# genomematt/xenomapper

Hardware: AMD Instinct MI355X
Metric: read-pairs/sec classified (higher is better)
Workload: dtype int32; 1 GPU; configs[1]: 50000000 PE 2x150 pairs/GPU, AS/XS, liberal, HBM-resident; pairs_per_gpu=50000000, step=xm_classify_compact_dev: classify+count, scan, scatter (3 launches)

## Files before the change

### xenomapper_amd/csrc/xm_api.hip

```cpp
#include <hip/hip_runtime.h>
#include <stdint.h>
#include <stdio.h>
#include <stdlib.h>
#include <string.h>

#include <dlfcn.h>

#include <string>
#include <vector>

#include <rccl/rccl.h>

#include "xm_kernels.h"
#include "xm_pinned.h"

struct TimedSpan {
    int kernel;
    hipEvent_t start, stop;
};

struct xm_ctx {
    int device;
    int n_cu;
    char name[128];
    uint32_t max_blocks;
    uint32_t *d_gran_counts;
    uint32_t *d_gran_off;
    uint64_t *d_counts_rep;
    uint32_t *d_part_tot;
    hipStream_t ws_stream;
    bool ws_used, ws_released;
    hipEvent_t ws_event;
    void *d_scratch[8];
    size_t scratch_bytes[8];
    bool timing;
    uint32_t timing_mask;
    std::vector<TimedSpan> spans;
    std::vector<hipEvent_t> free_events;
    double acc_ms[XM_K_COUNT];
    uint64_t acc_launches[XM_K_COUNT];
    std::string last_error;
    ncclComm_t comm;
    int comm_ranks;
// ... 112 lines not shown
int order_workspace(xm_ctx *ctx, hipStream_t st)
{
    if (capturing(st)) return XM_OK;
    if (ctx->ws_released) {
        XM_HIP(ctx, hipStreamWaitEvent(st, ctx->ws_event, 0));
        ctx->ws_released = false;
    } else if (ctx->ws_used && ctx->ws_stream != st && !capturing(ctx->ws_stream)) {
        XM_HIP(ctx, hipEventRecord(ctx->ws_event, ctx->ws_stream));
        XM_HIP(ctx, hipStreamWaitEvent(st, ctx->ws_event, 0));
    }
    ctx->ws_stream = st;
    ctx->ws_used = true;
    return XM_OK;
}

}

extern "C" {

int xm_abi_version(void) { return XM_ABI_VERSION; }

const char *xm_strerror(int status)
{
    switch (status) {
    case XM_OK: return "ok";
    case XM_ERR_INVALID_ARG: return "invalid argument";
    case XM_ERR_NO_DEVICE: return "no usable gfx950 (MI355X) device";
    case XM_ERR_HIP: return "HIP runtime error";
    case XM_ERR_OOM: return "out of device memory";
    case XM_ERR_RANGE: return "CIGAR-derived score outside int32";
// ... 17 lines not shown
    if (strncmp(prop.gcnArchName, "gfx950", 6) != 0) {
        char buf[200];
        snprintf(buf, sizeof buf, "device %d is %s, not gfx950", device_id, prop.gcnArchName);
        return no_device(buf, hipSuccess);
    }
    if ((he = hipSetDevice(device_id)) != hipSuccess) return no_device("hipSetDevice", he);

    xm_ctx *ctx = new xm_ctx();
    ctx->device = device_id;
    ctx->n_cu = prop.multiProcessorCount;
    snprintf(ctx->name, sizeof ctx->name, "%s (%s)", prop.name, prop.gcnArchName);
    ctx->max_blocks = (uint32_t)ctx->n_cu * 8u;
    ctx->d_gran_counts = nullptr;
    ctx->d_gran_off = nullptr;
    ctx->d_counts_rep = nullptr;
    ctx->d_part_tot = nullptr;
    ctx->ws_stream = nullptr;
    ctx->ws_used = false;
    ctx->ws_released = false;
    ctx->ws_event = nullptr;
    for (int i = 0; i < 8; ++i) { ctx->d_scratch[i] = nullptr; ctx->scratch_bytes[i] = 0; }
    ctx->timing = false;
    ctx->comm = nullptr;
    ctx->comm_ranks = 0;
    ctx->timing_mask = ~0u;
    for (int k = 0; k < XM_K_COUNT; ++k) { ctx->acc_ms[k] = 0.0; ctx->acc_launches[k] = 0; }
    const size_t ws = ((size_t)XM_MAX_GRANULES + 64) * 8 * sizeof(uint32_t);
    hipError_t e = hipMalloc((void **)&ctx->d_gran_counts, ws);
    if (e == hipSuccess) e = hipMalloc((void **)&ctx->d_gran_off, ws);
    if (e == hipSuccess) e = hipMalloc((void **)&ctx->d_counts_rep, COUNTS_REP_BYTES);
// ... 16 lines not shown
}

int xm_ctx_destroy(xm_ctx *ctx)
{
    if (!ctx) return XM_ERR_INVALID_ARG;
    (void)hipSetDevice(ctx->device);
    (void)hipDeviceSynchronize();
    if (ctx->comm) (void)xm_comm_destroy(ctx);
    for (auto &sp : ctx->spans) { (void)hipEventDestroy(sp.start); (void)hipEventDestroy(sp.stop); }
    for (auto &e : ctx->free_events) (void)hipEventDestroy(e);
    for (int i = 0; i < 8; ++i)
        if (ctx->d_scratch[i]) (void)hipFree(ctx->d_scratch[i]);
    (void)hipFree(ctx->d_gran_counts);
    (void)hipFree(ctx->d_gran_off);
    (void)hipFree(ctx->d_counts_rep);
    (void)hipFree(ctx->d_part_tot);
    (void)hipEventDestroy(ctx->ws_event);
    delete ctx;
    return XM_OK;
}

int xm_ctx_device_info(const xm_ctx *ctx, int *n_cu, char *name, size_t name_len)
{
    if (!ctx) return XM_ERR_INVALID_ARG;
    if (n_cu) *n_cu = ctx->n_cu;
    if (name && name_len) snprintf(name, name_len, "%s", ctx->name);
    return XM_OK;
}


// ... 109 lines not shown
        xm::launch_scan(st, cp, ctx->d_gran_off, bin_totals, counts);
    }
    if ((rc = check_launch(ctx, "scan_kernel")) != XM_OK) {
        reset_count_state(ctx, st);
        return rc;
    }
    {
        Span span(ctx, st, XM_K_SCATTER);
        xm::launch_scatter(st, cp.plan, mode, n, from_bins4 ? cp.bins4 : code, from_bins4, cp.gran_counts, ctx->d_gran_off,
                           bin_totals, bin_offsets, idx_out, ctx->d_part_tot, lists, cp.gran0, cp.gran1);
    }
    if ((rc = check_launch(ctx, "scatter_kernel")) != XM_OK) reset_count_state(ctx, st);
    return rc;
}

static xm::CountPlan count_plan(xm_ctx *ctx, uint64_t n)
{
    xm::CountPlan cp;
    cp.plan = xm::plan_granules(n);
    cp.gran_counts = ctx->d_gran_counts;
    cp.counts_rep = ctx->d_counts_rep;
    cp.part_tot = ctx->d_part_tot;
    cp.bins4 = nullptr;
    return cp;
}

static int empty_compact(xm_ctx *ctx, hipStream_t st, uint64_t *bin_offsets, uint64_t *counts)
{
    XM_HIP(ctx, hipMemsetAsync(counts, 0, 64 * sizeof(uint64_t), st));
    XM_HIP(ctx, hipMemsetAsync(bin_offsets, 0, 8 * sizeof(uint64_t), st));
    return XM_OK;
}

int xm_compact_dev(xm_ctx *ctx, void *stream, int mode, uint64_t n, const uint8_t *code,
                   uint32_t *idx_out, uint64_t *bin_offsets, uint64_t *counts)
{
    if (!ctx || bad_mode(mode) || n > XM_MAX_RECORDS || wrong_device(ctx)) return XM_ERR_INVALID_ARG;
    if (!bin_offsets || !counts) return XM_ERR_INVALID_ARG;
    hipStream_t st = (hipStream_t)stream;
    if (n == 0) return empty_compact(ctx, st, bin_offsets, counts);
    if (!code || !idx_out || ((uintptr_t)code & 15u)) return XM_ERR_INVALID_ARG;
    const xm::CountPlan cp = count_plan(ctx, n);
    int rc;
    if ((rc = order_workspace(ctx, st)) != XM_OK) return rc;
    {
        Span span(ctx, st, XM_K_HIST);
        xm::launch_hist(st, mode, n, code, cp);
    }
    if ((rc = check_launch(ctx, "hist_kernel")) != XM_OK) return rc;
    return compact_tail(ctx, st, mode, n, code, cp, idx_out, bin_offsets, counts);
}


int xm_classify_compact_dev(xm_ctx *ctx, void *stream, int mode, uint64_t n,
                            const int32_t *as1, const int32_t *xs1, const int32_t *as2, const int32_t *xs2,
                            const uint64_t *unit_bits, int32_t min_score_floor, uint8_t *code_out, uint8_t *bins4,
                            uint32_t *idx_out, uint64_t *bin_offsets, uint64_t *counts)
{
    if (!ctx || bad_mode(mode) || n > XM_MAX_RECORDS || wrong_device(ctx)) return XM_ERR_INVALID_ARG;
    if (!bin_offsets || !counts) return XM_ERR_INVALID_ARG;
    hipStream_t st = (hipStream_t)stream;
    if (n == 0) return empty_compact(ctx, st, bin_offsets, counts);
    if (!as1 || !xs1 || !as2 || !xs2 || !unit_bits || (!code_out && !bins4) || !idx_out) return XM_ERR_INVALID_ARG;
    if ((((uintptr_t)as1 | (uintptr_t)xs1 | (uintptr_t)as2 | (uintptr_t)xs2 | (uintptr_t)code_out | (uintptr_t)bins4) & 15u))
        return XM_ERR_INVALID_ARG;
    xm::CountPlan cp = count_plan(ctx, n);
    cp.bins4 = bins4;
    int rc;
    if ((rc = order_workspace(ctx, st)) != XM_OK) return rc;
    {
        Span span(ctx, st, XM_K_CLASSIFY);
        xm::launch_classify_i32(st, mode, n, as1, xs1, as2, xs2, unit_bits, min_score_floor, code_out, &cp);
    }
    if ((rc = check_launch(ctx, "classify_kernel<int32, counts>")) != XM_OK) return rc;
    return compact_tail(ctx, st, mode, n, code_out, cp, idx_out, bin_offsets, counts);
}

int xm_classify_compact_f64_dev(xm_ctx *ctx, void *stream, int mode, uint64_t n,
                                const double *as1, const double *xs1, const double *as2, const double *xs2,
                                const uint64_t *unit_bits, double min_score, uint8_t *code_out, uint8_t *bins4,
                                uint32_t *idx_out, uint64_t *bin_offsets, uint64_t *counts)
{
    if (!ctx || bad_mode(mode) || n > XM_MAX_RECORDS || wrong_device(ctx)) return XM_ERR_INVALID_ARG;
    if (!bin_offsets || !counts) return XM_ERR_INVALID_ARG;
    hipStream_t st = (hipStream_t)stream;
    if (n == 0) return empty_compact(ctx, st, bin_offsets, counts);
    if (!as1 || !xs1 || !as2 || !xs2 || !unit_bits || (!code_out && !bins4) || !idx_out) return XM_ERR_INVALID_ARG;
    if ((((uintptr_t)as1 | (uintptr_t)xs1 | (uintptr_t)as2 | (uintptr_t)xs2) & 31u) || (((uintptr_t)code_out | (uintptr_t)bins4) & 15u))
        return XM_ERR_INVALID_ARG;
    xm::CountPlan cp = count_plan(ctx, n);
    cp.bins4 = bins4;
    int rc;
    if ((rc = order_workspace(ctx, st)) != XM_OK) return rc;
    {
        Span span(ctx, st, XM_K_CLASSIFY);
        xm::launch_classify_f64(st, mode, n, as1, xs1, as2, xs2, unit_bits, min_score, code_out, &cp);
    }
    if ((rc = check_launch(ctx, "classify_kernel<f64, counts>")) != XM_OK) return rc;
    return compact_tail(ctx, st, mode, n, code_out, cp, idx_out, bin_offsets, counts);
}

int xm_classify_compact_cigar_dev(xm_ctx *ctx, void *stream, int mode, uint64_t n,
                                  const int32_t *nm1, const uint32_t *off1, const uint32_t *ops1, const int32_t *xs1,
                                  const int32_t *nm2, const uint32_t *off2, const uint32_t *ops2, const int32_t *xs2,
                                  const uint64_t *unit_bits, int32_t min_score_floor, uint8_t *code_out,
                                  uint32_t *range_flag, uint32_t *idx_out, uint64_t *bin_offsets, uint64_t *counts)
{
    if (!ctx || bad_mode(mode) || n > XM_MAX_RECORDS || wrong_device(ctx)) return XM_ERR_INVALID_ARG;
// ... 21 lines not shown
                                         const int32_t *nm2, const uint8_t *cnt2, const uint32_t *tile2, const uint32_t *ops2,
                                         const int32_t *xs2,
                                         const uint64_t *unit_bits, int32_t min_score_floor, uint8_t *code_out, uint8_t *bins4,
                                         uint32_t *range_flag, uint32_t *idx_out, uint64_t *bin_offsets, uint64_t *counts)
{
    if (!ctx || bad_mode(mode) || n > XM_MAX_RECORDS || wrong_device(ctx)) return XM_ERR_INVALID_ARG;
    if (!bin_offsets || !counts) return XM_ERR_INVALID_ARG;
    hipStream_t st = (hipStream_t)stream;
    if (n == 0) return empty_compact(ctx, st, bin_offsets, counts);
    if (!nm1 || !cnt1 || !tile1 || !ops1 || !xs1 || !nm2 || !cnt2 || !tile2 || !ops2 || !xs2 || !unit_bits ||
        (!code_out && !bins4) || !idx_out)
        return XM_ERR_INVALID_ARG;
    if ((((uintptr_t)nm1 | (uintptr_t)xs1 | (uintptr_t)nm2 | (uintptr_t)xs2 | (uintptr_t)code_out | (uintptr_t)bins4) & 15u) ||
        (((uintptr_t)cnt1 | (uintptr_t)cnt2 | (uintptr_t)tile1 | (uintptr_t)tile2 | (uintptr_t)ops1 | (uintptr_t)ops2) & 3u))
        return XM_ERR_INVALID_ARG;
    xm::CountPlan cp = count_plan(ctx, n);
    cp.bins4 = bins4;
    const xm::CigCols s1 = {nm1, xs1, cnt1, tile1, ops1}, s2 = {nm2, xs2, cnt2, tile2, ops2};
    int rc;
    if ((rc = order_workspace(ctx, st)) != XM_OK) return rc;
    {
        Span span(ctx, st, XM_K_CLASSIFY);
        xm::launch_classify_cigp(st, mode, n, s1, s2, unit_bits, min_score_floor, code_out, range_flag, cp);
    }
    if ((rc = check_launch(ctx, "classify_cigp_kernel")) != XM_OK) return rc;
    return compact_tail(ctx, st, mode, n, code_out, cp, idx_out, bin_offsets, counts);
}


static int list_out(uint32_t *const idx_out[6], uint32_t *idx_state6, uint64_t list_capacity, xm::ListOut &lo)
{
    if (!idx_out) return XM_ERR_INVALID_ARG;
    for (int b = 0; b < 6; ++b) {
        if (!idx_out[b] || ((uintptr_t)idx_out[b] & 3u)) return XM_ERR_INVALID_ARG;
        lo.p[b] = idx_out[b];
// ... 41 lines not shown
int xm_classify_place_dev(xm_ctx *ctx, void *stream, int mode, uint64_t n,
                          const int32_t *as1, const int32_t *xs1, const int32_t *as2, const int32_t *xs2,
                          const uint64_t *unit_bits, int32_t min_score_floor, uint8_t *code_out, uint8_t *bins4,
                          uint32_t *const idx_out[6], uint64_t list_capacity, uint64_t *n_out, uint64_t *counts)
{
    if (!ctx || bad_mode(mode) || n > XM_MAX_RECORDS || wrong_device(ctx)) return XM_ERR_INVALID_ARG;
    if (!n_out || !counts) return XM_ERR_INVALID_ARG;
    xm::ListOut lo;
    int rc;
    if ((rc = list_out(idx_out, nullptr, list_capacity, lo)) != XM_OK) return rc;
    hipStream_t st = (hipStream_t)stream;
    if (n == 0) return empty_compact(ctx, st, n_out, counts);
    if (!as1 || !xs1 || !as2 || !xs2 || !unit_bits || (!code_out && !bins4)) return XM_ERR_INVALID_ARG;
    if ((((uintptr_t)as1 | (uintptr_t)xs1 | (uintptr_t)as2 | (uintptr_t)xs2 | (uintptr_t)code_out | (uintptr_t)bins4) & 15u))
        return XM_ERR_INVALID_ARG;
    xm::CountPlan cp = count_plan(ctx, n);
    cp.bins4 = bins4;
    if ((rc = order_workspace(ctx, st)) != XM_OK) return rc;
    return place_steps(ctx, st, mode, n, cp, code_out, lo, n_out, counts, "classify_kernel<int32, counts>", [&](const xm::CountPlan &c) {
        xm::launch_classify_i32(st, mode, n, as1, xs1, as2, xs2, unit_bits, min_score_floor, code_out, &c);
    });
}

int xm_classify_place_f64_dev(xm_ctx *ctx, void *stream, int mode, uint64_t n,
                              const double *as1, const double *xs1, const double *as2, const double *xs2,
                              const uint64_t *unit_bits, double min_score, uint8_t *code_out, uint8_t *bins4,
                              uint32_t *const idx_out[6], uint32_t *idx_state6, uint64_t list_capacity,
                              uint64_t *n_out, uint64_t *counts)
{
    if (!ctx || bad_mode(mode) || n > XM_MAX_RECORDS || wrong_device(ctx)) return XM_ERR_INVALID_ARG;
    if (!n_out || !counts) return XM_ERR_INVALID_ARG;
    xm::ListOut lo;
    int rc;
    if ((rc = list_out(idx_out, idx_state6, list_capacity, lo)) != XM_OK) return rc;
    hipStream_t st = (hipStream_t)stream;
    if (n == 0) return empty_compact(ctx, st, n_out, counts);
    if (!as1 || !xs1 || !as2 || !xs2 || !unit_bits || (!code_out && !bins4)) return XM_ERR_INVALID_ARG;
    if ((((uintptr_t)as1 | (uintptr_t)xs1 | (uintptr_t)as2 | (uintptr_t)xs2) & 31u) || (((uintptr_t)code_out | (uintptr_t)bins4) & 15u))
        return XM_ERR_INVALID_ARG;
    xm::CountPlan cp = count_plan(ctx, n);
    cp.bins4 = bins4;
    if ((rc = order_workspace(ctx, st)) != XM_OK) return rc;
    return place_steps(ctx, st, mode, n, cp, code_out, lo, n_out, counts, "classify_kernel<f64, counts>", [&](const xm::CountPlan &c) {
        xm::launch_classify_f64(st, mode, n, as1, xs1, as2, xs2, unit_bits, min_score, code_out, &c);
    });
}

int xm_classify_place_cigar_packed_dev(xm_ctx *ctx, void *stream, int mode, uint64_t n,
                                       const int32_t *nm1, const uint8_t *cnt1, const uint32_t *tile1, const uint32_t *ops1,
                                       const int32_t *xs1,
                                       const int32_t *nm2, const uint8_t *cnt2, const uint32_t *tile2, const uint32_t *ops2,
                                       const int32_t *xs2,
                                       const uint64_t *unit_bits, int32_t min_score_floor, uint8_t *code_out, uint8_t *bins4,
                                       uint32_t *range_flag, uint32_t *const idx_out[6], uint64_t list_capacity,
                                       uint64_t *n_out, uint64_t *counts)
{
    if (!ctx || bad_mode(mode) || n > XM_MAX_RECORDS || wrong_device(ctx)) return XM_ERR_INVALID_ARG;
    if (!n_out || !counts) return XM_ERR_INVALID_ARG;
    xm::ListOut lo;
    int rc;
    if ((rc = list_out(idx_out, nullptr, list_capacity, lo)) != XM_OK) return rc;
    hipStream_t st = (hipStream_t)stream;
    if (n == 0) return empty_compact(ctx, st, n_out, counts);
    if (!nm1 || !cnt1 || !tile1 || !ops1 || !xs1 || !nm2 || !cnt2 || !tile2 || !ops2 || !xs2 || !unit_bits || (!code_out && !bins4))
        return XM_ERR_INVALID_ARG;
    if ((((uintptr_t)nm1 | (uintptr_t)xs1 | (uintptr_t)nm2 | (uintptr_t)xs2 | (uintptr_t)code_out | (uintptr_t)bins4) & 15u) ||
        (((uintptr_t)cnt1 | (uintptr_t)cnt2 | (uintptr_t)tile1 | (uintptr_t)tile2 | (uintptr_t)ops1 | (uintptr_t)ops2) & 3u))
        return XM_ERR_INVALID_ARG;
    xm::CountPlan cp = count_plan(ctx, n);
    cp.bins4 = bins4;
    const xm::CigCols s1 = {nm1, xs1, cnt1, tile1, ops1}, s2 = {nm2, xs2, cnt2, tile2, ops2};
    if ((rc = order_workspace(ctx, st)) != XM_OK) return rc;
    {
        Span span(ctx, st, XM_K_CLASSIFY);
        xm::launch_classify_cigp(st, mode, n, s1, s2, unit_bits, min_score_floor, code_out, range_flag, cp);
    }
    if ((rc = check_launch(ctx, "classify_cigp_kernel")) != XM_OK) return rc;
    return compact_tail(ctx, st, mode, n, code_out, cp, nullptr, n_out, counts, &lo);
}


static int runs_common(xm_ctx *ctx, hipStream_t st, int mode, uint64_t n, size_t elem,
                       const void *as1, const void *xs1, const void *as2, const void *xs2, const uint64_t *unit_bits,
                       int32_t mi, double mf, uint16_t *runs16, uint16_t *gran_counts, uint64_t *n_out, uint64_t *counts)
{
    if (!ctx || bad_mode(mode) || n > XM_MAX_RECORDS || wrong_device(ctx)) return XM_ERR_INVALID_ARG;
    if (!n_out || !counts) return XM_ERR_INVALID_ARG;
// ... 139 lines not shown
    XM_HIP(ctx, hipSetDevice(ctx->device));
    const size_t col_bytes = (size_t)n * elem;
    const size_t bits_bytes = (size_t)((n + 63) / 64) * 8;
    const void *src[4] = {as1, xs1, as2, xs2};
    int rc;
    for (int c = 0; c < 4; ++c) {
        if ((rc = ensure_scratch(ctx, c, col_bytes)) != XM_OK) return rc;
        XM_HIP(ctx, hipMemcpy(ctx->d_scratch[c], src[c], col_bytes, hipMemcpyHostToDevice));
    }
    if ((rc = ensure_scratch(ctx, 4, bits_bytes)) != XM_OK) return rc;
    XM_HIP(ctx, hipMemcpy(ctx->d_scratch[4], unit_bits, bits_bytes, hipMemcpyHostToDevice));
    if ((rc = ensure_scratch(ctx, 5, (size_t)n + 16)) != XM_OK) return rc;
    if ((rc = ensure_scratch(ctx, 7, 72 * sizeof(uint64_t))) != XM_OK) return rc;
    uint8_t *d_code = (uint8_t *)ctx->d_scratch[5];
    uint64_t *d_counts = (uint64_t *)ctx->d_scratch[7] + 8;
    const xm::CountPlan cp = count_plan(ctx, n);
    if (counts && (rc = order_workspace(ctx, nullptr)) != XM_OK) return rc;
    {
        Span span(ctx, nullptr, XM_K_CLASSIFY);
        if (elem == 4)
            xm::launch_classify_i32(nullptr, mode, n, (const int32_t *)ctx->d_scratch[0], (const int32_t *)ctx->d_scratch[1],
                                    (const int32_t *)ctx->d_scratch[2], (const int32_t *)ctx->d_scratch[3],
                                    (const uint64_t *)ctx->d_scratch[4], mi, d_code, counts ? &cp : nullptr);
        else
            xm::launch_classify_f64(nullptr, mode, n, (const double *)ctx->d_scratch[0], (const double *)ctx->d_scratch[1],
                                    (const double *)ctx->d_scratch[2], (const double *)ctx->d_scratch[3],
                                    (const uint64_t *)ctx->d_scratch[4], mf, d_code, counts ? &cp : nullptr);
    }
    if ((rc = check_launch(ctx, "classify_kernel")) != XM_OK) return rc;
    if (counts) {
        if ((rc = counts_only_tail(ctx, cp, d_counts)) != XM_OK) return rc;
        XM_HIP(ctx, hipMemcpy(counts, d_counts, 64 * sizeof(uint64_t), hipMemcpyDeviceToHost));
// ... 531 lines not shown
```

### xenomapper_amd/csrc/xm_kernels.h

```cpp
#pragma once
#include <hip/hip_runtime.h>
#include <stdint.h>

#include "../../include/xenomapper_hip.h"

#define XM_BLOCK 256
#define XM_GRAN 2048
#define XM_MAX_GRANULES ((uint32_t)((0xFFFFF000ull + XM_GRAN - 1) / XM_GRAN))
#define XM_PART_GRAN 1024u
#define XM_PART_STRIDE 2112u
#define XM_PART_REPLICAS 64u
#define XM_COUNT_REPLICAS 64u
#define XM_CLASSIFY_BLOCK 512
#ifndef XM_CIGAR_BLOCK
#define XM_CIGAR_BLOCK 256
#endif
#define XM_CIGP_BLOCK 512
#ifndef XM_SCATTER_WAVES
#define XM_SCATTER_WAVES 1048576u
#endif
#define XM_CLASSIFY_NT true

namespace xm {

struct GranPlan {
    uint32_t n_gran;
    uint32_t gran_stride;
};

struct CountPlan {
    GranPlan plan = {0, 0};
    uint32_t *gran_counts = nullptr;
    uint32_t *part_tot = nullptr;
    uint8_t *bins4 = nullptr;
    uint64_t *counts_rep = nullptr;
    uint32_t gran0 = 0, gran1 = 0;
};

GranPlan plan_granules(uint64_t n);

struct CigCols {
    const int32_t *nm;
    const int32_t *xs;
    const uint8_t *cnt;
    const uint32_t *tile;
    const uint32_t *ops;
};

struct ListOut {
    uint32_t *p[7];
// ... 41 lines not shown
```

### xenomapper_amd/csrc/xm_kernels.hip

```cpp
#include <hip/hip_runtime.h>
#include <stdint.h>
#include <stdlib.h>

#include "xm_kernels.h"

namespace xm {

template <typename T>
__device__ __forceinline__ uint32_t mapping_state(T a1, T x1, T a2, T x2, T m)
{
    const bool low1 = a1 <= m;
    const bool low2 = a2 <= m;
    const bool prim = (a1 > m) && (low2 || a1 > a2);
    const bool sec  = (a2 > m) && (low1 || a2 > a1);
    const bool spec1 = (x1 == T(0)) || (a1 > x1);
    const bool spec2 = (x2 == T(0)) || (a2 > x2);
    uint32_t s = 6u;
    s = sec ? (spec2 ? 1u : 3u) : s;
    s = (a1 == a2) ? 4u : s;
    s = prim ? (spec1 ? 0u : 2u) : s;
    s = (low1 && low2) ? 5u : s;
    return s;
}

// ... 79 lines not shown
{
    return (uint32_t)__builtin_amdgcn_readlane((int)v, lane);
}

__device__ __forceinline__ void lds_settle()
{
    asm volatile("s_waitcnt lgkmcnt(0)" ::: "memory");
}

#define XM_HREP 8
#define XM_COUNT_LDS_WORDS (64 * XM_HREP + 16)

struct CountSink {
    uint32_t *gran_counts;
    uint32_t *part_tot;
    unsigned long long *counts_rep;
    uint8_t *bins4;
    uint32_t gran_stride;
    int mode;
    uint32_t blk0;
};

__device__ __forceinline__ void count_flush(uint32_t *lds, uint32_t granule, const CountSink &sink)
{
    const uint32_t lane = threadIdx.x & 63u;
    uint32_t *misc = lds + 64 * XM_HREP;
    const uint4 h0 = *reinterpret_cast<const uint4 *>(lds + lane * XM_HREP);
    const uint4 h1 = *reinterpret_cast<const uint4 *>(lds + lane * XM_HREP + 4);
    const uint32_t s = h0.x + h0.y + h0.z + h0.w + h1.x + h1.y + h1.z + h1.w;
    if (s != 0u) {
        atomicAdd(&sink.counts_rep[(granule % XM_COUNT_REPLICAS) * 64u + lane], (unsigned long long)s);
        atomicAdd(&misc[8u + bin_of_code(sink.mode, lane)], s);
    }
    lds_settle();
    if (lane < 8u) {
        const uint32_t v = misc[8u + lane];
        sink.gran_counts[(uint64_t)lane * sink.gran_stride + granule] = v;
        if (v != 0u) atomicAdd(&sink.part_tot[((granule & (XM_PART_REPLICAS - 1u)) * 8u + lane) * XM_PART_STRIDE + granule / XM_PART_GRAN], v);
    }
}

template <int BLOCK>
__device__ __forceinline__ void count_units(const uint32_t c[4], uint32_t *lds, const CountSink &sink)
{
    const uint32_t lane = threadIdx.x & 63u;
    const uint32_t rep = lane & (XM_HREP - 1u);
#pragma unroll
    for (int j = 0; j < 4; ++j) {
// ... 221 lines not shown
{
    v += __shfl_xor(v, 1, 64);  v += __shfl_xor(v, 2, 64);  v += __shfl_xor(v, 4, 64);
    v += __shfl_xor(v, 8, 64);  v += __shfl_xor(v, 16, 64); v += __shfl_xor(v, 32, 64);
    if ((threadIdx.x & 63u) == 0u) wsum[threadIdx.x >> 6] = v;
    __syncthreads();
    unsigned long long total = 0;
#pragma unroll
    for (int w = 0; w < XM_SCAN_THREADS / 64; ++w) total += wsum[w];
    return total;
}

__global__ void __launch_bounds__(XM_SCAN_THREADS)
scan_kernel(const uint32_t *__restrict__ gran_counts, uint32_t n_gran, uint32_t gran_stride,
            const uint32_t *__restrict__ part_tot, uint32_t *__restrict__ gran_off,
            unsigned long long *__restrict__ bin_totals,
            unsigned long long *__restrict__ counts_rep, unsigned long long *__restrict__ counts, uint32_t part0, uint32_t n_parts)
{
    __shared__ unsigned long long wsum[XM_SCAN_THREADS / 64];
    __shared__ uint32_t wtot[XM_SCAN_THREADS / 64];
    const uint32_t p = blockIdx.x + part0, b = blockIdx.y;
    const uint32_t t = threadIdx.x, lane = t & 63u, wave = t >> 6;
    if (p + 1u == n_parts && t < 64u) {
        const uint32_t slot = b * 8u + (t >> 3), part = t & 7u;
        unsigned long long acc = 0;
        for (uint32_t r = part; r < XM_COUNT_REPLICAS; r += 8u) {
            acc += counts_rep[r * 64u + slot];
            counts_rep[r * 64u + slot] = 0;
        }
        acc += __shfl_xor(acc, 1, 64);
        acc += __shfl_xor(acc, 2, 64);
        acc += __shfl_xor(acc, 4, 64);
        if (part == 0) counts[slot] = acc;
    }
    const uint32_t g = p * XM_PART_GRAN + t;
    const uint32_t x = (g < n_gran) ? gran_counts[(uint64_t)b * gran_stride + g] : 0u;
    unsigned long long part_sum = 0;
    for (uint32_t e = t; e < p * XM_PART_REPLICAS; e += XM_SCAN_THREADS) {
        const uint32_t r = e / p, q = e - r * p;
        part_sum += part_tot[(r * 8u + b) * XM_PART_STRIDE + q];
    }
    const unsigned long long carry = block_sum_1024(part_sum, wsum);

    const uint32_t incl = wave_scan_incl(x);
    if (lane == 63u) wtot[wave] = incl;
    __syncthreads();
    uint32_t before_wave = 0, part_total = 0;
    for (uint32_t w = 0; w < XM_SCAN_THREADS / 64; ++w) {
        const uint32_t v = wtot[w];
        before_wave += (w < wave) ? v : 0u;
        part_total += v;
    }
    if (g < n_gran) gran_off[(uint64_t)b * gran_stride + g] = (uint32_t)carry + before_wave + incl - x;
    if (p + 1u == n_parts && t == 0u) bin_totals[b] = carry + part_total;
}

#ifndef XM_SCATTER_GUARD
// ... 169 lines not shown
    __shared__ __attribute__((aligned(16))) uint16_t slab_all[CAN_STAGE ? XM_BLOCK / 64 : 1][CAN_STAGE ? XM_SLAB_U16 : 4];
    const uint32_t lane = threadIdx.x & 63u;
    if (last) {
        const uint32_t n_parts = (n_gran + XM_PART_GRAN - 1u) / XM_PART_GRAN, cells = 8u * XM_PART_REPLICAS * n_parts;
        for (uint32_t i = blockIdx.x * XM_BLOCK + threadIdx.x; i < cells; i += gridDim.x * XM_BLOCK)
            part_tot[(i / n_parts) * XM_PART_STRIDE + i % n_parts] = 0u;
    }
    const uint32_t wave = (uint32_t)__builtin_amdgcn_readfirstlane((int)(threadIdx.x >> 6));
    const uint32_t g0 = g_first + (blockIdx.x * (XM_BLOCK / 64) + wave) * (MULTI ? gran_per_wave : 1u);
    if (g0 >= n_gran) return;
    uint8_t *lut = lut_all[NIB ? 0 : wave];
    if (!NIB) lut[lane] = (uint8_t)bin_of_code(mode, lane == 63u ? XM_NO_UNIT : lane);
    uint64_t *lptr = lptr_all[LISTS ? wave : 0];
    if (LISTS && lane < 8u) lptr[lane] = lane < 7u ? (uint64_t)(uintptr_t)lo.p[lane] : 0ull;

    uint32_t lane_base, n_units;
    {
        const uint32_t tot = (lane < 8u) ? (uint32_t)bin_totals[lane] : 0u;
        const uint32_t off = (lane < 7u) ? gran_off[(uint64_t)lane * gran_stride + g0] : 0u;
        const uint32_t bin_start = wave_scan_incl(tot) - tot;
        lane_base = LISTS ? off : bin_start + off;
        n_units = LISTS ? lo.cap : lane_value(bin_start, 7);
        if (g0 == g_first && last && lane < 8u) bin_offsets[lane] = (LISTS && lane < 7u) ? tot : bin_start;
    }
    uint16_t *slab = slab_all[CAN_STAGE ? wave : 0];

    auto load_granule = [&](uint32_t g, uint32_t w[NSUB]) {
        const uint64_t rec_g = (uint64_t)g * (NSUB * 256u);
        if (NIB) {
            const uint16_t *nib = reinterpret_cast<const uint16_t *>(code) + (rec_g >> 2) + lane;
#pragma unroll
            for (int s = 0; s < NSUB; ++s) w[s] = nib[s * 64];
        } else if (rec_g + NSUB * 256u <= n) {
#pragma unroll
            for (int s = 0; s < NSUB; ++s) w[s] = *reinterpret_cast<const uint32_t *>(code + rec_g + s * 256u + lane * 4u);
        } else {
#pragma unroll
            for (int s = 0; s < NSUB; ++s) w[s] = load_codes4_tail(code, rec_g + s * 256u + lane * 4u, n);
        }
    };
    auto slab_layout = [&](uint32_t cnt_g, uint32_t &run_start, uint32_t &run_len) -> bool {
        const uint32_t room = (lane < 7u) ? ((cnt_g + 3u) & ~3u) + 4u : 0u;
        const uint32_t incl_room = wave_scan_incl(room), incl_cnt = wave_scan_incl(cnt_g);
        run_start = incl_room - room + (lane_base & 3u);
        const uint32_t cnt = lane_base < n_units ? (cnt_g < n_units - lane_base ? cnt_g : n_units - lane_base) : 0u;
        run_len = run_start < (uint32_t)XM_SLAB_U16 ? (cnt < XM_SLAB_U16 - run_start ? cnt : XM_SLAB_U16 - run_start) : 0u;
        return lane_value(incl_cnt, 6) >= (uint32_t)XM_STAGE_MIN_UNITS;
    };
    auto copy_runs_out = [&](uint32_t run_start, uint32_t run_len, uint32_t rec_g) {
#pragma unroll
        for (int b = 0; b < 7; ++b) {
            const uint32_t N = lane_value(run_len, b);
            uint32_t *__restrict__ dst = LISTS ? lo.p[b] : idx_out;
            if (N == 0u || dst == nullptr) continue;
            scatter_copy_out<WIDE>(slab, lane_value(run_start, b), lane_value(lane_base, b), N, rec_g, dst);
        }
    };

    if (!MULTI) {
        const uint32_t g = g0;
        uint32_t run_start = 0, run_len = 0;
        bool staged = false;
        if (CAN_STAGE) {
            const uint32_t cnt_g = (lane < 7u) ? gran_counts[(uint64_t)lane * gran_stride + g] : 0u;
            staged = slab_layout(cnt_g, run_start, run_len);
        }
        uint32_t base[7];
#pragma unroll
        for (int b = 0; b < 7; ++b) base[b] = lane_value(staged ? run_start : lane_base, b);
        const uint32_t rec_g = (uint32_t)((uint64_t)g * (NSUB * 256u));
        uint32_t w[NSUB];
        load_granule(g, w);
        if (!NIB || LISTS) lds_settle();
        if (CAN_STAGE && staged) {
            scatter_granule<NSUB, WIDE, NIB, true, LISTS>(w, lut, rec_g, base, idx_out, n_units, slab, lptr);
            lds_settle();
            copy_runs_out(run_start, run_len, rec_g);
        } else {
            scatter_granule<NSUB, WIDE, NIB, false, LISTS>(w, lut, rec_g, base, idx_out, n_units, slab, lptr);
        }
        return;
    }

    const uint32_t g1 = g0 + gran_per_wave < n_gran ? g0 + gran_per_wave : n_gran;
    uint32_t base[7];
#pragma unroll
    for (int b = 0; b < 7; ++b) base[b] = lane_value(lane_base, b);
    uint32_t w[NSUB], wn[NSUB];
    load_granule(g0, w);
    if (!NIB || LISTS) lds_settle();
    for (uint32_t g = g0; g < g1; ++g) {
        if (g + 1u < g1) load_granule(g + 1u, wn);
        const uint32_t rec_g = (uint32_t)((uint64_t)g * (NSUB * 256u));
        bool staged = false;
        uint32_t cnt_g = 0;
        if (CAN_STAGE) {
            cnt_g = (lane < 7u) ? gran_counts[(uint64_t)lane * gran_stride + g] : 0u;
            uint32_t run_start, run_len;
            staged = slab_layout(cnt_g, run_start, run_len);
            if (staged) {
                uint32_t sbase[7];
#pragma unroll
                for (int b = 0; b < 7; ++b) sbase[b] = lane_value(run_start, b);
                scatter_granule<NSUB, WIDE, NIB, true, LISTS>(w, lut, rec_g, sbase, idx_out, n_units, slab, lptr);
                lds_settle();
                copy_runs_out(run_start, run_len, rec_g);
                lds_settle();
            }
        }
        if (!staged) {
            if (CAN_STAGE) {
#pragma unroll
// ... 433 lines not shown
#pragma unroll
        for (int j = 0; j < 4; ++j) a1[j] = a2[j] = INT32_MIN;
    }
    if (__ballot(bad) != 0ull && (threadIdx.x & 63u) == 0u && range_flag) atomicOr(range_flag, 1u);

    uint32_t halo = 0;
    if (PAIRED && threadIdx.x == 0) {
        if (r0 > 0) {
            const uint64_t h = r0 - 1;
            halo = mapping_state<int32_t>(cigar_score_one(nm1, off1, ops1, h, range_flag), xs1[h],
                                          cigar_score_one(nm2, off2, ops2, h, range_flag), xs2[h], m);
        } else {
            mb &= ~1u;
        }
    }
    const CountSink none = {nullptr, nullptr, nullptr, nullptr, 0u, 0, 0u};
    classify_finish<int32_t, PAIRED, BLOCK, FULL, false, -1>(a1, x1, a2, x2, m, mb, halo, last_state, code, r0, n, nullptr, none);
}

template <bool PAIRED, int BLOCK>
__global__ void __launch_bounds__(BLOCK)
classify_cigar_kernel(const int32_t *__restrict__ nm1, const uint32_t *__restrict__ off1, const uint32_t *__restrict__ ops1,
                      const int32_t *__restrict__ xs1,
                      const int32_t *__restrict__ nm2, const uint32_t *__restrict__ off2, const uint32_t *__restrict__ ops2,
                      const int32_t *__restrict__ xs2,
                      const uint8_t *__restrict__ unit_bits8, int32_t m, uint8_t *__restrict__ code, uint64_t n,
                      uint32_t *__restrict__ range_flag)
{
    __shared__ uint32_t last_state[BLOCK / 64];
    __shared__ __attribute__((aligned(16))) uint32_t cig_table[BLOCK / 64][XM_CIG_WAVE_OPS + 4];
    uint32_t *cig_T = cig_table[threadIdx.x >> 6];
// ... 334 lines not shown
GranPlan plan_granules(uint64_t n)
{
    GranPlan p;
    uint64_t g = (n + XM_GRAN - 1) / XM_GRAN;
    if (g == 0) g = 1;
    p.n_gran = (uint32_t)g;
    p.gran_stride = (p.n_gran + 63u) & ~63u;
    return p;
}

static CountSink make_sink(const CountPlan *cp, int mode)
{
    CountSink s;
    s.gran_counts = cp ? cp->gran_counts : nullptr;
    s.part_tot = cp ? cp->part_tot : nullptr;
    s.counts_rep = cp ? reinterpret_cast<unsigned long long *>(cp->counts_rep) : nullptr;
    s.bins4 = cp ? cp->bins4 : nullptr;
    s.gran_stride = cp ? cp->plan.gran_stride : 0u;
    s.mode = mode;
    s.blk0 = cp ? cp->gran0 : 0u;
    return s;
}

template <typename T>
static void launch_classify_t(hipStream_t st, int mode, uint64_t n,
                              const T *as1, const T *xs1, const T *as2, const T *xs2,
                              const uint64_t *unit_bits, T m, uint8_t *code, const CountPlan *cp)
{
    const uint64_t per_block = (uint64_t)XM_CLASSIFY_BLOCK * 4;
    static_assert(XM_CLASSIFY_BLOCK * 4 == XM_GRAN, "a counting workgroup is a granule: CountPlan's chunk is in both");
    const uint32_t all = (uint32_t)((n + per_block - 1) / per_block);
// ... 99 lines not shown
        if (mode == XM_MODE_SE) XM_LAUNCH_CIGP(false, -1); else XM_LAUNCH_CIGP(true, -1);
    }
#undef XM_LAUNCH_CIGP
}

void launch_hist(hipStream_t st, int mode, uint64_t n, const uint8_t *code, const CountPlan &cp)
{
    const uint32_t grid = (cp.plan.n_gran + (XM_BLOCK / 64) - 1) / (XM_BLOCK / 64);
    hist_kernel<<<grid, XM_BLOCK, 0, st>>>(code, n, cp.plan.n_gran, make_sink(&cp, mode));
}

void launch_scan(hipStream_t st, const CountPlan &cp, uint32_t *gran_off, uint64_t *bin_totals, uint64_t *counts)
{
    const uint32_t n_parts = (cp.plan.n_gran + XM_PART_GRAN - 1) / XM_PART_GRAN;
    unsigned long long *bt = reinterpret_cast<unsigned long long *>(bin_totals);
    unsigned long long *rep = reinterpret_cast<unsigned long long *>(cp.counts_rep);
    unsigned long long *cnt = reinterpret_cast<unsigned long long *>(counts);
    const uint32_t part0 = cp.gran1 ? cp.gran0 / XM_PART_GRAN : 0u;
    const uint32_t part1 = cp.gran1 ? (cp.gran1 + XM_PART_GRAN - 1) / XM_PART_GRAN : n_parts;
    scan_kernel<<<dim3(part1 - part0, 8), XM_SCAN_THREADS, 0, st>>>(cp.gran_counts, cp.gran1 ? cp.gran1 : cp.plan.n_gran, cp.plan.gran_stride,
                                                                   cp.part_tot, gran_off, bt, rep, cnt, part0, n_parts);
}

static uint32_t scatter_waves()
{
    const char *e = getenv("XM_SCATTER_WAVES");
    const long v = e && *e ? strtol(e, nullptr, 10) : 0;
    return v >= 1 && v < (long)XM_SCATTER_WAVES ? (uint32_t)v : (uint32_t)XM_SCATTER_WAVES;
}

void launch_scatter(hipStream_t st, const GranPlan &p, int mode, uint64_t n, const uint8_t *code, bool code_is_bins4,
                    const uint32_t *gran_counts, const uint32_t *gran_off, const uint64_t *bin_totals, uint64_t *bin_offsets,
                    uint32_t *idx_out, uint32_t *part_tot, const ListOut *lists, uint32_t gran0, uint32_t gran1)
{
    const unsigned long long *bt = reinterpret_cast<const unsigned long long *>(bin_totals);
    unsigned long long *bo = reinterpret_cast<unsigned long long *>(bin_offsets);
// ... 39 lines not shown
```

Baseline: 141.8 billion read-pairs/s.

## Replace replicated 64-bit count atomics with per-granule category rows reduced in scan

The classify/count epilogue no longer does a global 64-bit atomicAdd into replicated count slots. Each granule now writes its 64 category counts as uint16 into a new per-granule workspace, and the scan kernel reduces those rows per partition with wave shuffles before one atomic per bin. The scatter kernel also hoists the first granule's code and count loads ahead of the bin-total setup so their latency overlaps. This trades global atomic contention for extra HBM traffic, a lazily grown workspace, and zeroing of counts by granule 0, which relies on classify finishing before scan.

```diff
diff --git a/xenomapper_amd/csrc/xm_api.hip b/xenomapper_amd/csrc/xm_api.hip
--- a/xenomapper_amd/csrc/xm_api.hip
+++ b/xenomapper_amd/csrc/xm_api.hip
@@ -27,6 +27,8 @@
     uint32_t *d_gran_counts;
     uint32_t *d_gran_off;
     uint64_t *d_counts_rep;
+    uint16_t *d_gran_cat;
+    uint32_t gran_cat_cap;
     uint32_t *d_part_tot;
     hipStream_t ws_stream;
     bool ws_used, ws_released;
@@ -169,6 +171,25 @@
     return XM_OK;
 }
 
+int claim_workspace(xm_ctx *ctx, hipStream_t st, xm::CountPlan &cp)
+{
+    if (cp.plan.n_gran > ctx->gran_cat_cap) {
+        if (capturing(st)) {
+            ctx->last_error = "the workspace must grow for this input: run the call once outside the capture first";
+            return XM_ERR_INVALID_ARG;
+        }
+        if (ctx->d_gran_cat) XM_HIP(ctx, hipFree(ctx->d_gran_cat));
+        ctx->d_gran_cat = nullptr;
+        ctx->gran_cat_cap = 0;
+        const uint64_t room = (uint64_t)cp.plan.n_gran + cp.plan.n_gran / 8u + 64u;
+        const uint32_t cap = room > XM_MAX_GRANULES ? XM_MAX_GRANULES : (uint32_t)room;
+        XM_HIP(ctx, hipMalloc((void **)&ctx->d_gran_cat, (size_t)cap * 64 * sizeof(uint16_t)));
+        ctx->gran_cat_cap = cap;
+    }
+    cp.gran_cat = ctx->d_gran_cat;
+    return order_workspace(ctx, st);
+}
+
 }
 
 extern "C" {
@@ -216,6 +237,8 @@
     ctx->d_gran_counts = nullptr;
     ctx->d_gran_off = nullptr;
     ctx->d_counts_rep = nullptr;
+    ctx->d_gran_cat = nullptr;
+    ctx->gran_cat_cap = 0;
     ctx->d_part_tot = nullptr;
     ctx->ws_stream = nullptr;
     ctx->ws_used = false;
@@ -262,6 +285,7 @@
     (void)hipFree(ctx->d_gran_counts);
     (void)hipFree(ctx->d_gran_off);
     (void)hipFree(ctx->d_counts_rep);
+    if (ctx->d_gran_cat) (void)hipFree(ctx->d_gran_cat);
     (void)hipFree(ctx->d_part_tot);
     (void)hipEventDestroy(ctx->ws_event);
     delete ctx;
@@ -401,12 +425,12 @@
     return rc;
 }
 
-static xm::CountPlan count_plan(xm_ctx *ctx, uint64_t n)
+static xm::CountPlan count_plan(xm_ctx *ctx, uint64_t n, uint64_t *counts)
 {
     xm::CountPlan cp;
     cp.plan = xm::plan_granules(n);
     cp.gran_counts = ctx->d_gran_counts;
-    cp.counts_rep = ctx->d_counts_rep;
+    cp.counts = counts;
     cp.part_tot = ctx->d_part_tot;
     cp.bins4 = nullptr;
     return cp;
@@ -427,9 +451,9 @@
     hipStream_t st = (hipStream_t)stream;
     if (n == 0) return empty_compact(ctx, st, bin_offsets, counts);
     if (!code || !idx_out || ((uintptr_t)code & 15u)) return XM_ERR_INVALID_ARG;
-    const xm::CountPlan cp = count_plan(ctx, n);
-    int rc;
-    if ((rc = order_workspace(ctx, st)) != XM_OK) return rc;
+    xm::CountPlan cp = count_plan(ctx, n, counts);
+    int rc;
+    if ((rc = claim_workspace(ctx, st, cp)) != XM_OK) return rc;
     {
         Span span(ctx, st, XM_K_HIST);
         xm::launch_hist(st, mode, n, code, cp);
@@ -451,10 +475,10 @@
     if (!as1 || !xs1 || !as2 || !xs2 || !unit_bits || (!code_out && !bins4) || !idx_out) return XM_ERR_INVALID_ARG;
     if ((((uintptr_t)as1 | (uintptr_t)xs1 | (uintptr_t)as2 | (uintptr_t)xs2 | (uintptr_t)code_out | (uintptr_t)bins4) & 15u))
         return XM_ERR_INVALID_ARG;
-    xm::CountPlan cp = count_plan(ctx, n);
+    xm::CountPlan cp = count_plan(ctx, n, counts);
     cp.bins4 = bins4;
     int rc;
-    if ((rc = order_workspace(ctx, st)) != XM_OK) return rc;
+    if ((rc = claim_workspace(ctx, st, cp)) != XM_OK) return rc;
     {
         Span span(ctx, st, XM_K_CLASSIFY);
         xm::launch_classify_i32(st, mode, n, as1, xs1, as2, xs2, unit_bits, min_score_floor, code_out, &cp);
@@ -475,10 +499,10 @@
     if (!as1 || !xs1 || !as2 || !xs2 || !unit_bits || (!code_out && !bins4) || !idx_out) return XM_ERR_INVALID_ARG;
     if ((((uintptr_t)as1 | (uintptr_t)xs1 | (uintptr_t)as2 | (uintptr_t)xs2) & 31u) || (((uintptr_t)code_out | (uintptr_t)bins4) & 15u))
         return XM_ERR_INVALID_ARG;
-    xm::CountPlan cp = count_plan(ctx, n);
+    xm::CountPlan cp = count_plan(ctx, n, counts);
     cp.bins4 = bins4;
     int rc;
-    if ((rc = order_workspace(ctx, st)) != XM_OK) return rc;
+    if ((rc = claim_workspace(ctx, st, cp)) != XM_OK) return rc;
     {
         Span span(ctx, st, XM_K_CLASSIFY);
         xm::launch_classify_f64(st, mode, n, as1, xs1, as2, xs2, unit_bits, min_score, code_out, &cp);
@@ -530,11 +554,11 @@
     if ((((uintptr_t)nm1 | (uintptr_t)xs1 | (uintptr_t)nm2 | (uintptr_t)xs2 | (uintptr_t)code_out | (uintptr_t)bins4) & 15u) ||
         (((uintptr_t)cnt1 | (uintptr_t)cnt2 | (uintptr_t)tile1 | (uintptr_t)tile2 | (uintptr_t)ops1 | (uintptr_t)ops2) & 3u))
         return XM_ERR_INVALID_ARG;
-    xm::CountPlan cp = count_plan(ctx, n);
+    xm::CountPlan cp = count_plan(ctx, n, counts);
     cp.bins4 = bins4;
     const xm::CigCols s1 = {nm1, xs1, cnt1, tile1, ops1}, s2 = {nm2, xs2, cnt2, tile2, ops2};
     int rc;
-    if ((rc = order_workspace(ctx, st)) != XM_OK) return rc;
+    if ((rc = claim_workspace(ctx, st, cp)) != XM_OK) return rc;
     {
         Span span(ctx, st, XM_K_CLASSIFY);
         xm::launch_classify_cigp(st, mode, n, s1, s2, unit_bits, min_score_floor, code_out, range_flag, cp);
@@ -606,9 +630,9 @@
     if (!as1 || !xs1 || !as2 || !xs2 || !unit_bits || (!code_out && !bins4)) return XM_ERR_INVALID_ARG;
     if ((((uintptr_t)as1 | (uintptr_t)xs1 | (uintptr_t)as2 | (uintptr_t)xs2 | (uintptr_t)code_out | (uintptr_t)bins4) & 15u))
         return XM_ERR_INVALID_ARG;
-    xm::CountPlan cp = count_plan(ctx, n);
+    xm::CountPlan cp = count_plan(ctx, n, counts);
     cp.bins4 = bins4;
-    if ((rc = order_workspace(ctx, st)) != XM_OK) return rc;
+    if ((rc = claim_workspace(ctx, st, cp)) != XM_OK) return rc;
     return place_steps(ctx, st, mode, n, cp, code_out, lo, n_out, counts, "classify_kernel<int32, counts>", [&](const xm::CountPlan &c) {
         xm::launch_classify_i32(st, mode, n, as1, xs1, as2, xs2, unit_bits, min_score_floor, code_out, &c);
     });
@@ -630,9 +654,9 @@
     if (!as1 || !xs1 || !as2 || !xs2 || !unit_bits || (!code_out && !bins4)) return XM_ERR_INVALID_ARG;
     if ((((uintptr_t)as1 | (uintptr_t)xs1 | (uintptr_t)as2 | (uintptr_t)xs2) & 31u) || (((uintptr_t)code_out | (uintptr_t)bins4) & 15u))
         return XM_ERR_INVALID_ARG;
-    xm::CountPlan cp = count_plan(ctx, n);
+    xm::CountPlan cp = count_plan(ctx, n, counts);
     cp.bins4 = bins4;
-    if ((rc = order_workspace(ctx, st)) != XM_OK) return rc;
+    if ((rc = claim_workspace(ctx, st, cp)) != XM_OK) return rc;
     return place_steps(ctx, st, mode, n, cp, code_out, lo, n_out, counts, "classify_kernel<f64, counts>", [&](const xm::CountPlan &c) {
         xm::launch_classify_f64(st, mode, n, as1, xs1, as2, xs2, unit_bits, min_score, code_out, &c);
     });
@@ -659,10 +683,10 @@
     if ((((uintptr_t)nm1 | (uintptr_t)xs1 | (uintptr_t)nm2 | (uintptr_t)xs2 | (uintptr_t)code_out | (uintptr_t)bins4) & 15u) ||
         (((uintptr_t)cnt1 | (uintptr_t)cnt2 | (uintptr_t)tile1 | (uintptr_t)tile2 | (uintptr_t)ops1 | (uintptr_t)ops2) & 3u))
         return XM_ERR_INVALID_ARG;
-    xm::CountPlan cp = count_plan(ctx, n);
+    xm::CountPlan cp = count_plan(ctx, n, counts);
     cp.bins4 = bins4;
     const xm::CigCols s1 = {nm1, xs1, cnt1, tile1, ops1}, s2 = {nm2, xs2, cnt2, tile2, ops2};
-    if ((rc = order_workspace(ctx, st)) != XM_OK) return rc;
+    if ((rc = claim_workspace(ctx, st, cp)) != XM_OK) return rc;
     {
         Span span(ctx, st, XM_K_CLASSIFY);
         xm::launch_classify_cigp(st, mode, n, s1, s2, unit_bits, min_score_floor, code_out, range_flag, cp);
@@ -832,8 +856,8 @@
     if ((rc = ensure_scratch(ctx, 7, 72 * sizeof(uint64_t))) != XM_OK) return rc;
     uint8_t *d_code = (uint8_t *)ctx->d_scratch[5];
     uint64_t *d_counts = (uint64_t *)ctx->d_scratch[7] + 8;
-    const xm::CountPlan cp = count_plan(ctx, n);
-    if (counts && (rc = order_workspace(ctx, nullptr)) != XM_OK) return rc;
+    xm::CountPlan cp = count_plan(ctx, n, d_counts);
+    if (counts && (rc = claim_workspace(ctx, nullptr, cp)) != XM_OK) return rc;
     {
         Span span(ctx, nullptr, XM_K_CLASSIFY);
         if (elem == 4)
diff --git a/xenomapper_amd/csrc/xm_kernels.h b/xenomapper_amd/csrc/xm_kernels.h
--- a/xenomapper_amd/csrc/xm_kernels.h
+++ b/xenomapper_amd/csrc/xm_kernels.h
@@ -33,7 +33,8 @@
     uint32_t *gran_counts = nullptr;
     uint32_t *part_tot = nullptr;
     uint8_t *bins4 = nullptr;
-    uint64_t *counts_rep = nullptr;
+    uint16_t *gran_cat = nullptr;
+    uint64_t *counts = nullptr;
     uint32_t gran0 = 0, gran1 = 0;
 };
 
diff --git a/xenomapper_amd/csrc/xm_kernels.hip b/xenomapper_amd/csrc/xm_kernels.hip
--- a/xenomapper_amd/csrc/xm_kernels.hip
+++ b/xenomapper_amd/csrc/xm_kernels.hip
@@ -117,7 +117,8 @@
 struct CountSink {
     uint32_t *gran_counts;
     uint32_t *part_tot;
-    unsigned long long *counts_rep;
+    uint16_t *gran_cat;
+    unsigned long long *counts;
     uint8_t *bins4;
     uint32_t gran_stride;
     int mode;
@@ -131,10 +132,9 @@
     const uint4 h0 = *reinterpret_cast<const uint4 *>(lds + lane * XM_HREP);
     const uint4 h1 = *reinterpret_cast<const uint4 *>(lds + lane * XM_HREP + 4);
     const uint32_t s = h0.x + h0.y + h0.z + h0.w + h1.x + h1.y + h1.z + h1.w;
-    if (s != 0u) {
-        atomicAdd(&sink.counts_rep[(granule % XM_COUNT_REPLICAS) * 64u + lane], (unsigned long long)s);
-        atomicAdd(&misc[8u + bin_of_code(sink.mode, lane)], s);
-    }
+    sink.gran_cat[(uint64_t)granule * 64u + lane] = (uint16_t)s;
+    if (granule == 0u) sink.counts[lane] = 0ull;
+    if (s != 0u) atomicAdd(&misc[8u + bin_of_code(sink.mode, lane)], s);
     lds_settle();
     if (lane < 8u) {
         const uint32_t v = misc[8u + lane];
@@ -386,32 +386,39 @@
 scan_kernel(const uint32_t *__restrict__ gran_counts, uint32_t n_gran, uint32_t gran_stride,
             const uint32_t *__restrict__ part_tot, uint32_t *__restrict__ gran_off,
             unsigned long long *__restrict__ bin_totals,
-            unsigned long long *__restrict__ counts_rep, unsigned long long *__restrict__ counts, uint32_t part0, uint32_t n_parts)
+            const uint16_t *__restrict__ gran_cat, unsigned long long *__restrict__ counts, uint32_t part0, uint32_t n_parts)
 {
     __shared__ unsigned long long wsum[XM_SCAN_THREADS / 64];
     __shared__ uint32_t wtot[XM_SCAN_THREADS / 64];
+    __shared__ uint32_t wcat[XM_SCAN_THREADS / 64][8];
     const uint32_t p = blockIdx.x + part0, b = blockIdx.y;
     const uint32_t t = threadIdx.x, lane = t & 63u, wave = t >> 6;
-    if (p + 1u == n_parts && t < 64u) {
-        const uint32_t slot = b * 8u + (t >> 3), part = t & 7u;
-        unsigned long long acc = 0;
-        for (uint32_t r = part; r < XM_COUNT_REPLICAS; r += 8u) {
-            acc += counts_rep[r * 64u + slot];
-            counts_rep[r * 64u + slot] = 0;
-        }
-        acc += __shfl_xor(acc, 1, 64);
-        acc += __shfl_xor(acc, 2, 64);
-        acc += __shfl_xor(acc, 4, 64);
-        if (part == 0) counts[slot] = acc;
-    }
     const uint32_t g = p * XM_PART_GRAN + t;
     const uint32_t x = (g < n_gran) ? gran_counts[(uint64_t)b * gran_stride + g] : 0u;
+    uint4 row = make_uint4(0u, 0u, 0u, 0u);
+    if (g < n_gran) row = *reinterpret_cast<const uint4 *>(gran_cat + (uint64_t)g * 64u + b * 8u);
+    {
+        uint32_t cat[8] = {row.x & 0xFFFFu, row.x >> 16, row.y & 0xFFFFu, row.y >> 16,
+                           row.z & 0xFFFFu, row.z >> 16, row.w & 0xFFFFu, row.w >> 16};
+#pragma unroll
+        for (int k = 0; k < 8; ++k) {
+#pragma unroll
+            for (int m = 1; m < 64; m <<= 1) cat[k] += __shfl_xor(cat[k], m, 64);
+            if (lane == 0u) wcat[wave][k] = cat[k];
+        }
+    }
     unsigned long long part_sum = 0;
     for (uint32_t e = t; e < p * XM_PART_REPLICAS; e += XM_SCAN_THREADS) {
         const uint32_t r = e / p, q = e - r * p;
         part_sum += part_tot[(r * 8u + b) * XM_PART_STRIDE + q];
     }
     const unsigned long long carry = block_sum_1024(part_sum, wsum);
+    if (t < 8u) {
+        unsigned long long sum = 0;
+#pragma unroll
+        for (int w = 0; w < XM_SCAN_THREADS / 64; ++w) sum += wcat[w][t];
+        if (sum != 0ull) atomicAdd(&counts[b * 8u + t], sum);
+    }
 
     const uint32_t incl = wave_scan_incl(x);
     if (lane == 63u) wtot[wave] = incl;
@@ -611,6 +618,25 @@
     uint64_t *lptr = lptr_all[LISTS ? wave : 0];
     if (LISTS && lane < 8u) lptr[lane] = lane < 7u ? (uint64_t)(uintptr_t)lo.p[lane] : 0ull;
 
+    auto load_granule = [&](uint32_t g, uint32_t w[NSUB]) {
+        const uint64_t rec_g = (uint64_t)g * (NSUB * 256u);
+        if (NIB) {
+            const uint16_t *nib = reinterpret_cast<const uint16_t *>(code) + (rec_g >> 2) + lane;
+#pragma unroll
+            for (int s = 0; s < NSUB; ++s) w[s] = nib[s * 64];
+        } else if (rec_g + NSUB * 256u <= n) {
+#pragma unroll
+            for (int s = 0; s < NSUB; ++s) w[s] = *reinterpret_cast<const uint32_t *>(code + rec_g + s * 256u + lane * 4u);
+        } else {
+#pragma unroll
+            for (int s = 0; s < NSUB; ++s) w[s] = load_codes4_tail(code, rec_g + s * 256u + lane * 4u, n);
+        }
+    };
+    uint32_t w[NSUB];
+    load_granule(g0, w);
+    uint32_t cnt_g0 = 0;
+    if (CAN_STAGE) cnt_g0 = (lane < 7u) ? gran_counts[(uint64_t)lane * gran_stride + g0] : 0u;
+
     uint32_t lane_base, n_units;
     {
         const uint32_t tot = (lane < 8u) ? (uint32_t)bin_totals[lane] : 0u;
@@ -622,20 +648,6 @@
     }
     uint16_t *slab = slab_all[CAN_STAGE ? wave : 0];
 
-    auto load_granule = [&](uint32_t g, uint32_t w[NSUB]) {
-        const uint64_t rec_g = (uint64_t)g * (NSUB * 256u);
-        if (NIB) {
-            const uint16_t *nib = reinterpret_cast<const uint16_t *>(code) + (rec_g >> 2) + lane;
-#pragma unroll
-            for (int s = 0; s < NSUB; ++s) w[s] = nib[s * 64];
-        } else if (rec_g + NSUB * 256u <= n) {
-#pragma unroll
-            for (int s = 0; s < NSUB; ++s) w[s] = *reinterpret_cast<const uint32_t *>(code + rec_g + s * 256u + lane * 4u);
-        } else {
-#pragma unroll
-            for (int s = 0; s < NSUB; ++s) w[s] = load_codes4_tail(code, rec_g + s * 256u + lane * 4u, n);
-        }
-    };
     auto slab_layout = [&](uint32_t cnt_g, uint32_t &run_start, uint32_t &run_len) -> bool {
         const uint32_t room = (lane < 7u) ? ((cnt_g + 3u) & ~3u) + 4u : 0u;
         const uint32_t incl_room = wave_scan_incl(room), incl_cnt = wave_scan_incl(cnt_g);
@@ -658,16 +670,11 @@
         const uint32_t g = g0;
         uint32_t run_start = 0, run_len = 0;
         bool staged = false;
-        if (CAN_STAGE) {
-            const uint32_t cnt_g = (lane < 7u) ? gran_counts[(uint64_t)lane * gran_stride + g] : 0u;
-            staged = slab_layout(cnt_g, run_start, run_len);
-        }
+        if (CAN_STAGE) staged = slab_layout(cnt_g0, run_start, run_len);
         uint32_t base[7];
 #pragma unroll
         for (int b = 0; b < 7; ++b) base[b] = lane_value(staged ? run_start : lane_base, b);
         const uint32_t rec_g = (uint32_t)((uint64_t)g * (NSUB * 256u));
-        uint32_t w[NSUB];
-        load_granule(g, w);
         if (!NIB || LISTS) lds_settle();
         if (CAN_STAGE && staged) {
             scatter_granule<NSUB, WIDE, NIB, true, LISTS>(w, lut, rec_g, base, idx_out, n_units, slab, lptr);
@@ -683,8 +690,7 @@
     uint32_t base[7];
 #pragma unroll
     for (int b = 0; b < 7; ++b) base[b] = lane_value(lane_base, b);
-    uint32_t w[NSUB], wn[NSUB];
-    load_granule(g0, w);
+    uint32_t wn[NSUB];
     if (!NIB || LISTS) lds_settle();
     for (uint32_t g = g0; g < g1; ++g) {
         if (g + 1u < g1) load_granule(g + 1u, wn);
@@ -692,7 +698,8 @@
         bool staged = false;
         uint32_t cnt_g = 0;
         if (CAN_STAGE) {
-            cnt_g = (lane < 7u) ? gran_counts[(uint64_t)lane * gran_stride + g] : 0u;
+            cnt_g = cnt_g0;
+            if (g != g0) cnt_g = (lane < 7u) ? gran_counts[(uint64_t)lane * gran_stride + g] : 0u;
             uint32_t run_start, run_len;
             staged = slab_layout(cnt_g, run_start, run_len);
             if (staged) {
@@ -1156,7 +1163,7 @@
             mb &= ~1u;
         }
     }
-    const CountSink none = {nullptr, nullptr, nullptr, nullptr, 0u, 0, 0u};
+    const CountSink none = {nullptr, nullptr, nullptr, nullptr, nullptr, 0u, 0, 0u};
     classify_finish<int32_t, PAIRED, BLOCK, FULL, false, -1>(a1, x1, a2, x2, m, mb, halo, last_state, code, r0, n, nullptr, none);
 }
 
@@ -1521,7 +1528,8 @@
     CountSink s;
     s.gran_counts = cp ? cp->gran_counts : nullptr;
     s.part_tot = cp ? cp->part_tot : nullptr;
-    s.counts_rep = cp ? reinterpret_cast<unsigned long long *>(cp->counts_rep) : nullptr;
+    s.gran_cat = cp ? cp->gran_cat : nullptr;
+    s.counts = cp ? reinterpret_cast<unsigned long long *>(cp->counts) : nullptr;
     s.bins4 = cp ? cp->bins4 : nullptr;
     s.gran_stride = cp ? cp->plan.gran_stride : 0u;
     s.mode = mode;
@@ -1651,12 +1659,11 @@
 {
     const uint32_t n_parts = (cp.plan.n_gran + XM_PART_GRAN - 1) / XM_PART_GRAN;
     unsigned long long *bt = reinterpret_cast<unsigned long long *>(bin_totals);
-    unsigned long long *rep = reinterpret_cast<unsigned long long *>(cp.counts_rep);
     unsigned long long *cnt = reinterpret_cast<unsigned long long *>(counts);
     const uint32_t part0 = cp.gran1 ? cp.gran0 / XM_PART_GRAN : 0u;
     const uint32_t part1 = cp.gran1 ? (cp.gran1 + XM_PART_GRAN - 1) / XM_PART_GRAN : n_parts;
     scan_kernel<<<dim3(part1 - part0, 8), XM_SCAN_THREADS, 0, st>>>(cp.gran_counts, cp.gran1 ? cp.gran1 : cp.plan.n_gran, cp.plan.gran_stride,
-                                                                   cp.part_tot, gran_off, bt, rep, cnt, part0, n_parts);
+                                                                   cp.part_tot, gran_off, bt, cp.gran_cat, cnt, part0, n_parts);
 }
 
 static uint32_t scatter_waves()
```

New measurement: 139.9 billion read-pairs/s. -1.3%, worse.
